# BlackCloud37/rust-raytracer

Hardware: AMD Instinct MI355X
Metric: Msamples/sec (px*spp), scene_500 1200x1200 1000spp (higher is better)
Workload: dtype f64

## Files before the change

### rust-raytracer_amd/csrc/device/kernels.hip

```cpp
#include <hip/hip_runtime.h>

#include <cmath>
#include <cstdio>
#include <chrono>
#include <cstdlib>
#include <cstring>
#include <map>
#include <memory>
#include <mutex>
#include <vector>

#include "../common/flat.h"
#include "../common/grid_shape.h"
#include "../common/detlog.h"
#include "../common/detsin.h"
#include "../common/detuv.h"
#include "../common/rng.h"
#include "../common/schedule.h"
#include "../common/tighten.h"
#include "device.h"

namespace rtamd {

#ifndef PT_BLOCK
#define PT_BLOCK 1024
#endif

#define HIP_CHECK(expr)                                                                                  \
    do {                                                                                                 \
        hipError_t _e = (expr);                                                                          \
        if (_e != hipSuccess)                                                                            \
            throw RtError((_e == hipErrorNoDevice || _e == hipErrorInvalidDevice) ? RT_ERR_NO_DEVICE : RT_ERR_HIP, \
                          std::string(#expr) + ": " + hipGetErrorString(_e));                            \
    } while (0)

#ifdef RTAMD_PHASE_STATS
__shared__ unsigned long long s_ph[48];
__device__ unsigned long long g_phase[48];
__device__ __forceinline__ bool ph_first() { return (int)(__ffsll((long long)__ballot(1)) - 1) == (int)(threadIdx.x & 63); }
#define PH_CLK() __builtin_amdgcn_s_memtime()
#define PH_ADD(i, dt)                                                         \
    do {                                                                      \
        if (ph_first()) atomicAdd(&s_ph[(i)], (unsigned long long)(dt));      \
    } while (0)
#define PH_EV(i)                                                              \
    do {                                                                      \
        const unsigned long long _m = __ballot(1);                            \
        if (ph_first()) {                                                     \
            atomicAdd(&s_ph[16 + (i)], 1ull);                                 \
            atomicAdd(&s_ph[32 + (i)], (unsigned long long)__popcll(_m));     \
        }                                                                     \
    } while (0)
#define PH_BEGIN(v) const unsigned long long v = PH_CLK()
#define PH_END(i, v)              \
    do {                          \
        PH_ADD(i, PH_CLK() - v);  \
        PH_EV(i);                 \
    } while (0)
#else
#define PH_ADD(i, dt) \
    do {              \
    } while (0)
#define PH_EV(i) \
    do {         \
    } while (0)
#define PH_BEGIN(v) \
    do {            \
    } while (0)
#define PH_END(i, v) \
    do {             \
    } while (0)
#endif

struct D3 {
    double x, y, z;
};
#define DEV __device__ __forceinline__
DEV D3 mk(double x, double y, double z) { D3 r; r.x = x; r.y = y; r.z = z; return r; }
DEV D3 add(D3 a, D3 b) { return mk(a.x + b.x, a.y + b.y, a.z + b.z); }
DEV D3 sub(D3 a, D3 b) { return mk(a.x - b.x, a.y - b.y, a.z - b.z); }
DEV D3 muls(D3 a, double s) { return mk(a.x * s, a.y * s, a.z * s); }
DEV D3 divs(D3 a, double s) { return mk(a.x / s, a.y / s, a.z / s); }
DEV D3 neg(D3 a) { return mk(-a.x, -a.y, -a.z); }
DEV D3 elemul(D3 a, D3 b) { return mk(a.x * b.x, a.y * b.y, a.z * b.z); }
DEV double dot(D3 a, D3 b) { return a.x * b.x + a.y * b.y + a.z * b.z; }
DEV double sqlen(D3 a) { return a.x * a.x + a.y * a.y + a.z * a.z; }
DEV D3 cross(D3 a, D3 b) { return mk(a.y * b.z - a.z * b.y, a.z * b.x - a.x * b.z, a.x * b.y - a.y * b.x); }
DEV double comp(D3 a, int i) { return i == 0 ? a.x : (i == 1 ? a.y : a.z); }
DEV D3 unit(D3 a, int* err) {
    double l = sqrt(sqlen(a));
    if (l == 0.) atomicOr(err, 1);
    return divs(a, l);
}
DEV bool near_zero(D3 a) {
    const double S = 1e-8;
    return (fabs(a.x) < S) && (fabs(a.y) < S) && (fabs(a.z) < S);
}
DEV D3 reflect(D3 v, D3 n) { return sub(v, muls(n, 2. * dot(v, n))); }
DEV D3 refract(D3 uv, D3 n, double eta) {
    double cos_theta = fmin(dot(neg(uv), n), 1.0);
    D3 perp = muls(add(uv, muls(n, cos_theta)), eta);
    D3 par = muls(n, -sqrt(fabs(1.0 - sqlen(perp))));
    return add(perp, par);
}
DEV D3 random_in_unit_sphere(Rng& rng) {
    double u, v, r2;
    for (;;) {
        u = rng.gen_range_pm1();
        v = rng.gen_range_pm1();
        r2 = u * u + v * v;
        if (r2 <= 1.) break;
    }
    double q = sqrt(1. - r2);
    return mk(2. * u * q, 2. * v * q, 1. - 2. * r2);
}
DEV D3 random_in_unit_disk(Rng& rng) {
    for (;;) {
        double a = rng.gen_range_pm1();
        double b = rng.gen_range_pm1();
        if (a * a + b * b + 0. * 0. >= 1.) continue;
        return mk(a, b, 0.);
    }
}
DEV D3 xf_point(const double* t, D3 p) {
    return mk(t[0] * p.x + t[1] * p.y + t[2] * p.z + t[3] * 1., t[4] * p.x + t[5] * p.y + t[6] * p.z + t[7] * 1.,
              t[8] * p.x + t[9] * p.y + t[10] * p.z + t[11] * 1.);
}
DEV D3 xf_dir(const double* t, D3 p) {
    return mk(t[0] * p.x + t[1] * p.y + t[2] * p.z + t[3] * 0., t[4] * p.x + t[5] * p.y + t[6] * p.z + t[7] * 0.,
              t[8] * p.x + t[9] * p.y + t[10] * p.z + t[11] * 0.);
}

#define AS_G __attribute__((address_space(1)))
// ... 1342 lines not shown
    const AreaTriDev* k = T + lo;
    double u = x2, v = x3;
    if (u + v > 1.0) {
        u = 1.0 - u;
        v = 1.0 - v;
    }
    const D3 p = add(mk(k->a[0], k->a[1], k->a[2]), add(muls(mk(k->e0[0], k->e0[1], k->e0[2]), u), muls(mk(k->e1[0], k->e1[1], k->e1[2]), v)));
    return sub(p, o);
}
__device__ __attribute__((noinline)) double area_pdf(const char* tab, uint32_t li, D3 o, D3 d) {
    const AreaTab a = area_tab(tab);
    const AreaLightDev l = a.lights[li];
    const double total = (double)l.total, d2 = sqlen(d), dl = sqrt(d2);
    double sum = 0.0;
    for (uint32_t i = 0; i < l.count; i++) {
        const AreaTriDev* k = a.tris + l.first + i;
        double t, b1, b2;
        if (!tri_hit_v(mk(k->a[0], k->a[1], k->a[2]), mk(k->e0[0], k->e0[1], k->e0[2]), mk(k->e1[0], k->e1[1], k->e1[2]), o, d, 0.001, INFINITY, t, b1, b2)) continue;
        const double area2 = k->area2;
        const double dist2 = (t * t) * d2;
        const double cosine = fabs(dot(d, mk(k->n[0], k->n[1], k->n[2])) / (dl * area2));
        if (!(cosine > 0.)) continue;
        sum = sum + (((double)k->q / total) * dist2) / (cosine * (0.5 * area2));
    }
    return sum;
}
DEV bool mixture_step_area(const Acc& A, const char* area, const char* env, const Rec& rec, Rng& rng, D3 att, D3& beta, D3& dir, int* err) {
    const double PI = 3.14159265358979323846264338327950288;
    const uint32_t M = ((const AreaHdr*)area)->n_lights;
    const uint32_t n = A.n_lights + M + (env ? 1u : 0u);
    if (rng.gen_f64() < 0.5) {
        uint32_t li = (uint32_t)(rng.gen_f64() * (double)n);
        if (li >= n) li = n - 1u;
        if (li < A.n_lights) {
            dir = light_random(A, A.lights[li], rec.p, rng, err);
        } else if (li < A.n_lights + M) {
            const double x1 = rng.gen_f64(), x2 = rng.gen_f64(), x3 = rng.gen_f64();
            dir = area_sample(area, li - A.n_lights, rec.p, x1, x2, x3);
        } else {
            const double x1 = rng.gen_f64(), x2 = rng.gen_f64(), x3 = rng.gen_f64(), x4 = rng.gen_f64();
            dir = env_sample(env, x1, x2, x3, x4);
        }
    }
    double cosine = dot(rec.normal, unit(dir, err));
    double scattering_pdf = (cosine < 0.) ? 0. : cosine / PI;
    double lp = 0.;
    for (uint32_t i = 0; i < A.n_lights; i++) lp = lp + light_pdf_value(A, A.lights[i], rec.p, dir);
    for (uint32_t i = 0; i < M; i++) lp = lp + area_pdf(area, i, rec.p, dir);
    if (env) lp = lp + env_pdf(env, dir, err);
    double pdf_val = 0.5 * (lp / (double)n) + 0.5 * scattering_pdf;
    double wgt = scattering_pdf / pdf_val;
    if (!(wgt > 0.)) return false;
    beta = muls(elemul(beta, att), wgt);
    return true;
}

#ifndef REGEN_MIN
#define REGEN_MIN 8
#endif
#ifndef FOLD_RETRY
#define FOLD_RETRY 4
#endif
#ifndef COOP_EARLY_FOLD
#define COOP_EARLY_FOLD 1
#endif
#ifndef POOL_MODE
#define POOL_MODE 1
#endif
#ifndef FOLD_BATCH
#define FOLD_BATCH 1
#endif
#ifndef FOLD_PERIOD
#define FOLD_PERIOD 4
#endif
#ifndef UNIT_SPP_N
#define UNIT_SPP_N 8
#endif
static const int UNIT_SPP = UNIT_SPP_N;
#ifndef RING_UNITS
#define RING_UNITS 8
#endif
static const int UNIT_DOUBLES = UNIT_SPP * TILE_PIX * 3;
static_assert(RING_UNITS * 4 <= 64, "a wave clears its ring bookkeeping with one store per lane");
#ifndef SINGLE_UNITS_BELOW_WAVES
#define SINGLE_UNITS_BELOW_WAVES 1
#endif
#ifndef JOB_UNITS
#define JOB_UNITS 2
#endif
DEV uint64_t ld_agent(const uint64_t* p) { return __hip_atomic_load(p, __ATOMIC_RELAXED, __HIP_MEMORY_SCOPE_AGENT); }
DEV void st_agent(uint64_t* p, uint64_t v) { __hip_atomic_store(p, v, __ATOMIC_RELAXED, __HIP_MEMORY_SCOPE_AGENT); }
DEV uint64_t ld_agent_g(const AS_G uint64_t* p) { return __hip_atomic_load(p, __ATOMIC_RELAXED, __HIP_MEMORY_SCOPE_AGENT); }
DEV void st_agent_g(AS_G uint64_t* p, uint64_t v) { __hip_atomic_store(p, v, __ATOMIC_RELAXED, __HIP_MEMORY_SCOPE_AGENT); }

#ifdef RT_TAIL_STATS
__device__ unsigned long long g_tail_end[8192], g_tail_beg[8192], g_tail_entry[8192];
__device__ unsigned int g_tail_xcc[8192];
#endif
#ifdef RT_FOLD_STATS
__device__ unsigned long long g_fold_stats[8];
#endif
__device__ __attribute__((noinline)) int fold_units(const uint32_t* rmeta, const double* wring, double* accum, unsigned int* tickets, bool first_launch,
                                                    int r_head, int r_cnt, bool idle, int lane, int ring_units) {
#ifdef RT_FOLD_STATS
    const unsigned long long t_in = __builtin_amdgcn_s_memtime();
    unsigned long long n_mis = 0, n_sleep = 0;
#endif
    const AS_L uint32_t* rm = (const AS_L uint32_t*)rmeta;
    AS_G unsigned int* tk_g = (AS_G unsigned int*)tickets;
    int folded = 0;
    bool have = false;
    uint32_t cur_tile = 0;
    double ax = 0., ay = 0., az = 0.;
    asm volatile("s_waitcnt vmcnt(0)" ::: "memory");
    while (r_cnt > 0) {
        const AS_L uint32_t* m = rm + 4 * r_head;
        if (__hip_atomic_load(&m[3], __ATOMIC_RELAXED, __HIP_MEMORY_SCOPE_WORKGROUP) != 0u) break;
        const uint32_t tile = m[0], blk = m[1], ns = m[2] & 0xffu;
        const bool first = (m[2] & 0x100u) != 0u, last = (m[2] & 0x200u) != 0u;
        if (first) {
            const uint32_t tk = __hip_atomic_load(&tk_g[tile], __ATOMIC_RELAXED, __HIP_MEMORY_SCOPE_AGENT);
            if (tk != blk) {
#ifdef RT_FOLD_STATS
                if (!idle) n_mis++;
                else n_sleep++;
#endif
                if (!idle) break;
                __builtin_amdgcn_s_sleep(4);
                continue;
            }
        }
        AS_G uint64_t* acc = (AS_G uint64_t*)accum + ((size_t)tile * TILE_PIX + (size_t)lane) * 3;
        if (!have) {
            ax = 0.; ay = 0.; az = 0.;
            if (!(blk == 0u && first_launch)) {
                ax = __longlong_as_double(ld_agent_g(acc));
                ay = __longlong_as_double(ld_agent_g(acc + 1));
                az = __longlong_as_double(ld_agent_g(acc + 2));
            }
            have = true;
            cur_tile = tile;
        }
        const AS_G uint64_t* p = (const AS_G uint64_t*)wring + ((size_t)r_head * UNIT_SPP * TILE_PIX + (size_t)lane) * 3;
        uint32_t si = 0;
#if FOLD_BATCH > 1
        for (; si + FOLD_BATCH <= ns; si += FOLD_BATCH) {
            uint64_t v[3 * FOLD_BATCH];
#pragma unroll
            for (int k = 0; k < 3 * FOLD_BATCH; k++) v[k] = ld_agent_g(p + (size_t)(k / 3) * (TILE_PIX * 3) + (k % 3));
#pragma unroll
            for (int j = 0; j < FOLD_BATCH; j++) {
                ax = ax + __longlong_as_double(v[3 * j]);
                ay = ay + __longlong_as_double(v[3 * j + 1]);
                az = az + __longlong_as_double(v[3 * j + 2]);
            }
            p += FOLD_BATCH * TILE_PIX * 3;
        }
#endif
        for (; si < ns; si++) {
            const uint64_t v0 = ld_agent_g(p), v1 = ld_agent_g(p + 1), v2 = ld_agent_g(p + 2);
            ax = ax + __longlong_as_double(v0);
            ay = ay + __longlong_as_double(v1);
            az = az + __longlong_as_double(v2);
            p += TILE_PIX * 3;
        }
        r_head = (r_head + 1 == ring_units) ? 0 : r_head + 1;
// ... 259 lines not shown
}

#ifndef RT_TIGHTEN_BOXES
#define RT_TIGHTEN_BOXES 1
#endif
static constexpr int INTEG_BG = 4;
static constexpr int INTEG_ENV = 8;
static constexpr int INTEG_AREA = 16;
template <bool LDS, int GENERAL, int ACCEL, int INTEG, bool MEDIA = false, bool POOL = false>
__global__ void __launch_bounds__(PT_BLOCK) pt_kernel(FlatView sv, CamK cam, RenderK rk, double* __restrict__ ring, double* accum,
                                                      unsigned int* tickets, unsigned int* __restrict__ counter, int* __restrict__ err) {
    extern __shared__ __attribute__((aligned(16))) char smem[];
#ifdef RT_TAIL_STATS
    const unsigned long long tail_entry = __builtin_amdgcn_s_memrealtime();
#endif
    const uint32_t st_begin = (ACCEL == 2) ? sv.stage2_begin : 0u;
    const uint32_t st_end = (ACCEL == 2) ? sv.stage2_end : sv.stage_bytes;
    uint32_t staged = 0;
    Acc A;
    if (LDS && ACCEL == 2) {
        const uint32_t lo_bytes = sv.off_n2 - st_begin;
        {
            const uint4* src = (const uint4*)(sv.base + st_begin);
            uint4* dst = (uint4*)smem;
            for (uint32_t i = threadIdx.x; i < lo_bytes / 16; i += blockDim.x) dst[i] = src[i];
        }
        char* n2w = smem + lo_bytes;
        stage_nodew(sv, n2w, rk.box_shrink);
        staged = lo_bytes + nodew_bytes(sv.n_nodes2);
        __syncthreads();
        A = make_acc(smem - st_begin, sv.base, sv);
        A.n2 = nullptr;
        A.n2w_lds = (uint32_t)(uintptr_t)(AS_L char*)n2w;
        if (MEDIA) {
            A.meta = (const uint2*)(sv.base + sv.off_meta);
            A.boxes = (const double2*)(sv.base + sv.off_boxes);
        }
    } else if (LDS) {
        const uint4* src = (const uint4*)(sv.base + st_begin);
        uint4* dst = (uint4*)smem;
        for (uint32_t i = threadIdx.x; i < (st_end - st_begin) / 16; i += blockDim.x) dst[i] = src[i];
        staged = st_end - st_begin;
        __syncthreads();
        A = make_acc(smem - st_begin, sv.base, sv);
    } else {
        A = make_acc(sv.base, sv.base, sv);
        if (ACCEL == 2 && rk.n_top > 0) {
            const uint4* src = (const uint4*)(sv.base + sv.off_n2);
            uint4* dst = (uint4*)smem;
            for (uint32_t i = threadIdx.x; i < (uint32_t)rk.n_top * NODE2_F4; i += blockDim.x) dst[i] = src[i];
            __syncthreads();
            A.n2_top = (const AS_L f32x4*)smem;
            A.n2_top_count = (uint32_t)rk.n_top;
            staged = (uint32_t)rk.n_top * (uint32_t)sizeof(Node2);
        }
    }
    const char* area_env = nullptr;
    if ((INTEG & INTEG_AREA) && sv.off_env != 0u && ((const EnvTabHdr*)(sv.base + sv.total_bytes))->total != 0ull) area_env = sv.base + sv.total_bytes;
    uint32_t* stk = (uint32_t*)(smem + staged) + threadIdx.x;
    const int stk_stride = (int)blockDim.x;
    const int lane = threadIdx.x & 63;
    const uint64_t lanemask_lt = (1ull << lane) - 1ull;
    const int wave = threadIdx.x >> 6;
    uint32_t* book = (uint32_t*)(smem + staged + walk_stack_bytes((ACCEL == 2) ? sv.stack2 : 0u, PT_BLOCK));
    uint32_t* rmeta = book + (size_t)wave * RING_UNITS * 4;
    uint32_t* wst = book + (size_t)(PT_BLOCK / 64) * RING_UNITS * 4 + (size_t)wave * 8;
    int* cfg = (int*)(book + (size_t)(PT_BLOCK / 64) * (RING_UNITS * 4 + 8));
    if (lane < 8) wst[lane] = (lane == 6) ? 1u : 0u;
    if (POOL && lane < RING_UNITS * 4) rmeta[lane] = 0u;
    if (threadIdx.x == 0) {
        cfg[CFG_N_JOBS] = rk.n_units; cfg[CFG_TILES_OWNED] = rk.tiles_owned; cfg[CFG_JOB_UNITS] = rk.job_units;
        cfg[CFG_SUBS_PER_TILE] = rk.subs_per_tile; cfg[CFG_WORLD] = rk.world; cfg[CFG_RANK] = rk.rank; cfg[CFG_TILES_X] = rk.tiles_x;
        cfg[CFG_S_BEGIN] = rk.s_begin; cfg[CFG_S_END] = rk.s_end; cfg[CFG_SUB_SPP] = rk.sub_spp; cfg[CFG_WIDTH] = rk.width;
        cfg[CFG_HEIGHT] = rk.height;
        cfg[CFG_RING_UNITS] = RING_UNITS;
        cfg[CFG_JOB_LISTS] = 1;
#pragma unroll
        for (int i = 0; i < 25; i++) cfg[CFG_LVL + i] = rk.lvl[i / 5][i % 5];
        cfg[CFG_TILE_LIST] = (int)(uint32_t)(uintptr_t)rk.tile_list; cfg[CFG_TILE_LIST + 1] = (int)(uint32_t)((uint64_t)(uintptr_t)rk.tile_list >> 32);
    }
    if (GENERAL >= 2 && rk.time_slots) A.time_lds = (uint32_t)(uintptr_t)(AS_L char*)(cfg + CFG_WORDS);
    __syncthreads();
    double* wring = ring + ((size_t)blockIdx.x * (PT_BLOCK / 64) + (size_t)wave) * RING_UNITS * UNIT_DOUBLES;

    int tx = 0, ty = 0, s0 = 0, pool = 0, next = 0, cur_slot = 0;
    bool finished = false;

    bool alive = false;
    D3 o = mk(0, 0, 0), d = mk(0, 0, 1), beta = mk(1, 1, 1), L = mk(0, 0, 0);
    int depth = 0;
    int pix_id = 0;
    uint32_t out_slot = 0;
    Rng rng;
    rng.s = 0;
#ifdef RT_TAIL_STATS
    const unsigned long long tail_t0 = __builtin_amdgcn_s_memrealtime();
#endif
    int fold_wait = 0;
#ifdef RTAMD_PHASE_STATS
    if (threadIdx.x < 48) s_ph[threadIdx.x] = 0ull;
    __syncthreads();
#endif
    {
        for (;;) {
            PH_BEGIN(ph_it0);
            uint64_t dead = __ballot(!alive);
            if ((int)__popcll(dead) < REGEN_MIN && dead != ~0ull) dead = 0ull;
            const bool need_unit = dead != 0ull && next >= pool && !finished;
            bool head_ready = false;
            if (FOLD_PERIOD > 0 && !need_unit && --fold_wait < 0) {
                fold_wait = FOLD_PERIOD - 1;
                head_ready = __builtin_amdgcn_readfirstlane(wst[1]) != 0u &&
                             __builtin_amdgcn_readfirstlane(__hip_atomic_load(&rmeta[4 * __builtin_amdgcn_readfirstlane(wst[0]) + 3], __ATOMIC_RELAXED,
                                                                              __HIP_MEMORY_SCOPE_WORKGROUP)) == 0u;
            }
            if (need_unit || head_ready) {
                const UnitInfo u = uniform_unit(POOL ? next_unit_pool(wst, rmeta, cfg, wring, accum, tickets, counter, need_unit && dead == ~0ull, lane, need_unit)
                                                     : next_unit(wst, rmeta, cfg, wring, accum, tickets, counter, need_unit && dead == ~0ull, lane, need_unit));
                if (need_unit) {
                    if (u.pool > 0) {
                        pool = u.pool;
                        next = 0;
                        s0 = u.s0;
                        tx = u.tx;
                        ty = u.ty;
                        cur_slot = u.cur_slot;
                    }
                    finished = u.finished != 0;
                } else if (u.cur_slot == 0) {
                    fold_wait = FOLD_RETRY;
                }
            }
            if (dead != 0ull && next < pool) {
                int k = next + __popcll(dead & lanemask_lt);
                next = min(next + (int)__popcll(dead), pool);
                if (!alive && k < pool) {
                    int pix = k & (TILE_PIX - 1), s = s0 + (k >> 6);
                    int x = tx * TILE_W + (pix & (TILE_W - 1)), y = ty * TILE_H + (pix >> 3);
                    if (x < rk.width && y < rk.height) {
                        rng.seed_stream(rk.seed, (uint64_t)y * (uint64_t)rk.width + (uint64_t)x, (uint64_t)s);
                        double u = ((double)x + rng.gen_f64()) / (double)(rk.width - 1);
                        double v = ((double)y + rng.gen_f64()) / (double)(rk.height - 1);
                        double st = 1.0 - v;
                        D3 rd = muls(random_in_unit_disk(rng), cam.lens_radius);
                        if (GENERAL >= 2 && rk.time1 > rk.time0) {
                            const double tm = rng.gen_range(rk.time0, rk.time1);
                            if (A.time_lds) *(AS_L double*)(uintptr_t)(A.time_lds + 8u * threadIdx.x) = tm;
                        } else if (GENERAL >= 2 && A.time_lds) {
                            *(AS_L double*)(uintptr_t)(A.time_lds + 8u * threadIdx.x) = rk.time0;
                        }
                        D3 offset = add(muls(cam.u, rd.x), muls(cam.v, rd.y));
                        o = add(cam.origin, offset);
                        d = sub(sub(add(add(cam.llc, muls(cam.horizontal, u)), muls(cam.vertical, st)), cam.origin), offset);
                        beta = mk(1., 1., 1.);
                        L = mk(0., 0., 0.);
                        depth = rk.max_depth;
                        pix_id = y * rk.width + x;
                        out_slot = ((uint32_t)cur_slot * (uint32_t)UNIT_SPP + (uint32_t)(k >> 6)) * (uint32_t)TILE_PIX + (uint32_t)pix;
                        alive = true;
                    }
                }
            }
            PH_END(0, ph_it0);
            if (__ballot(alive) == 0ull && next >= pool && finished) break;
            if (alive) {
                PH_EV(13);
                PH_BEGIN(ph_t0);
                Hit h = (ACCEL == 2) ? (MEDIA ? traverse2_media<GENERAL, !LDS, LDS>(A, sv.n_media, stk, stk_stride, o, d, rk.t_min, rng)
                                              : traverse2<GENERAL, false, !LDS, LDS>(A, stk, stk_stride, o, d, rk.t_min, INFINITY))
                                     : traverse<GENERAL, MEDIA>(A, o, d, rk.t_min, INFINITY, &rng);
                PH_END(1, ph_t0);
                PH_BEGIN(ph_p0);
                bool done = true;
                if (h.node >= 0 && depth > 0) {
                    depth -= 1;
                    PH_BEGIN(ph_m0);
                    const Rec rec = materialize<GENERAL>(A, h, o, d, err);
                    PH_END(2, ph_m0);
                    constexpr bool SEG_IN_PLACE = !(GENERAL == 1 && !LDS && ACCEL == 2 && INTEG == INTEG_BG && MEDIA) &&
                                                  !(GENERAL == 3 && LDS && ACCEL == 1 && INTEG == (INTEG_BG | 1));
                    if (SEG_IN_PLACE) o = rec.p;
                    D3 emitted, att, ndir = d;
                    D3& nd = SEG_IN_PLACE ? d : ndir;
                    bool diffuse, scattered;
                    PH_BEGIN(ph_s0);
                    if constexpr (GENERAL == 0) {
                        const auto add_emitted = [&](const D3& le) {
                            L = add(L, elemul(beta, le));
                            asm volatile("" : "+v"(L.x), "+v"(L.y), "+v"(L.z));
                        };
                        scattered = shade<GENERAL>(A, rec, d, rng, emitted, att, nd, diffuse, err, add_emitted);
                    } else {
                        scattered = shade<GENERAL>(A, rec, d, rng, emitted, att, nd, diffuse, err);
                        L = add(L, elemul(beta, emitted));
                    }
                    PH_END(3, ph_s0);
                    if (scattered) {
                        if ((INTEG & 3) == 2 && diffuse) {
                            const double* e = rk.sppm_est + 6 * (size_t)pix_id;
                            L = add(L, elemul(beta, mk(e[0], e[1], e[2])));
                            L = add(L, elemul(beta, mk(e[3], e[4], e[5])));
                        } else if ((INTEG & 3) == 1 && diffuse) {
                            PH_EV(14);
                            if (INTEG & INTEG_AREA) done = !mixture_step_area(A, sv.base + sv.off_area, area_env, rec, rng, att, beta, nd, err);
                            else if (INTEG & INTEG_ENV) done = !mixture_step_env(A, sv.base + sv.total_bytes, rec, rng, att, beta, nd, err);
                            else done = !mixture_step(A, rec, rng, att, beta, nd, err);
                        } else {
                            beta = elemul(beta, att);
                            done = false;
                        }
                        if (!SEG_IN_PLACE && !done) {
                            o = rec.p;
                            d = ndir;
                        }
                    }
                } else if ((INTEG & INTEG_BG) && h.node < 0 && (!(INTEG & INTEG_AREA) || sv.off_bg != 0u)) {
                    L = add(L, elemul(beta, background_radiance<GENERAL>((const BgDev*)(sv.base + sv.off_bg), A.texs, A.texels, d, err)));
                }
                if (done) {
                    double* dst = wring + 3 * (size_t)out_slot;
                    dst[0] = L.x;
                    dst[1] = L.y;
                    dst[2] = L.z;
                    atomicSub(rmeta + 4 * (out_slot >> 9) + 3, 1u);
                    alive = false;
                }
                PH_END(8, ph_p0);
            }
        }
    }
#ifdef RTAMD_PHASE_STATS
    __syncthreads();
    if (threadIdx.x < 48) atomicAdd(&g_phase[threadIdx.x], s_ph[threadIdx.x]);
#endif
#ifdef RT_TAIL_STATS
    if (lane == 0) {
        g_tail_end[blockIdx.x * (PT_BLOCK / 64) + wave] = __builtin_amdgcn_s_memrealtime();
        g_tail_beg[blockIdx.x * (PT_BLOCK / 64) + wave] = tail_t0;
        g_tail_entry[blockIdx.x * (PT_BLOCK / 64) + wave] = tail_entry;
        g_tail_xcc[blockIdx.x * (PT_BLOCK / 64) + wave] = 0u;
    }
#endif
}

#ifndef COOP_POOL
#define COOP_POOL 1024
#endif
#define COOP_RING (2 * COOP_POOL)
static_assert(COOP_RING >= 2 * COOP_POOL && COOP_POOL <= 32768 && (COOP_RING & (COOP_RING - 1)) == 0,
              "kernel 5's rings: 16-bit entries (id + 1), power-of-two capacity of at least twice the pool (see ring_pop)");
#ifndef COOP_SPIN_MAX
#define COOP_SPIN_MAX (1u << 16)
#endif
#ifndef COOP_BATCH
#define COOP_BATCH 32
#endif
#ifndef COOP_REFILL_TH
#define COOP_REFILL_TH 56
#endif
#ifndef COOP_ENTRY_NODES
#define COOP_ENTRY_NODES 64
#endif
#ifndef COOP_ADOPT_MIN
#define COOP_ADOPT_MIN 8
#endif
#ifndef COOP_SUSPEND_TH
#define COOP_SUSPEND_TH 24
#endif
static const int COOP_MAX_INST = 64;
static const int COOP_STACK_MAX = 40;
static const int COOP_REC = 20 + COOP_STACK_MAX / 2 + 2;
typedef unsigned long long U2 __attribute__((ext_vector_type(2)));
DEV U2 ld_unit(const uint64_t* rec, int unit) { return ((const U2*)rec)[unit]; }
DEV void st_unit(uint64_t* rec, int unit, uint64_t a, uint64_t b) {
    U2 v;
    v.x = a;
    v.y = b;
    ((U2*)rec)[unit] = v;
}
DEV uint64_t dbits(double x) { return (uint64_t)__double_as_longlong(x); }
DEV double bitsd(uint64_t x) { return __longlong_as_double((long long)x); }

#ifdef RTAMD_COOP_STATS
__device__ unsigned long long g_coop_stats[16];
struct CoopStats {
    unsigned long long ev[8] = {0, 0, 0, 0, 0, 0, 0, 0}, ln[8] = {0, 0, 0, 0, 0, 0, 0, 0};
    unsigned long long tm[8] = {0, 0, 0, 0, 0, 0, 0, 0}, t_last = 0;
};
__device__ unsigned long long g_coop_time[8];
#define COOP_RING_T0 const unsigned long long t_ring0 = __builtin_amdgcn_s_memtime()
#define COOP_RING_T1 cs.tm[7] += __builtin_amdgcn_s_memtime() - t_ring0
#define COOP_TIME(i)                                                      \
    do {                                                                  \
        const unsigned long long t_now = __builtin_amdgcn_s_memtime();    \
        cs.tm[i] += t_now - cs.t_last;                                    \
        cs.t_last = t_now;                                                \
    } while (0)
#define COOP_STATS_ARG , CoopStats& cs
#define COOP_STATS_PASS , cs
#define COOP_STAT(i, lanes_mask)                                        \
    do {                                                                \
        cs.ev[i] += 1ull;                                               \
        cs.ln[i] += (unsigned long long)__popcll(lanes_mask);           \
    } while (0)
#else
#define COOP_STATS_ARG
#define COOP_STATS_PASS
#define COOP_STAT(i, lanes_mask) \
    do {                         \
    } while (0)
#define COOP_TIME(i) \
    do {             \
    } while (0)
#define COOP_RING_T0
#define COOP_RING_T1
#endif
// ... 1558 lines not shown
    if (kernel == 0)
        kernel = accel2_usable ? ((coop_usable && view.max_inst_nodes2 >= 64u) ? 5 : (wf_usable && !coop_usable && view.max_inst_nodes2 >= 64u) ? 6 : 2) : 1;
    if (kernel == 5 && !coop_usable)
        throw RtError(RT_ERR_UNSUPPORTED, "kernel 5 (cooperative instance service) needs a usable accel, 1..64 instances of which at least one holds only triangles with f32 vertices (an OBJ mesh), of BVH depth <= 40");
    if (kernel == 6 && !wf_usable)
        throw RtError(RT_ERR_UNSUPPORTED, "kernel 6 (wavefront instance service) needs a usable accel and 1..64 instances of which at least one holds only triangles with f32 vertices (an OBJ mesh)");
    if ((kernel == 2 || kernel == 5) && !accel2_usable)
        throw RtError(RT_ERR_UNSUPPORTED, "kernel 2 requested but no usable accel for this scene/camera (unbounded item, depth overflow, stacks "
                                          "larger than LDS, negative t_min, or camera farther than 64x the scene extent); use kernel 0/1");
    c.kernel = kernel;
    const size_t ring_meta = ((size_t)(PT_BLOCK / 64) * (RING_UNITS * 4 + 8) + CFG_WORDS) * sizeof(uint32_t);
    c.stack_bytes = ((kernel == 2) ? stack2_bytes : (kernel == 5) ? stack5_bytes : 0) + ring_meta + ((kernel == 5) ? coop_lds : 0);
    if (plan.tile_list && !plan.ext_accum) throw RtError(RT_ERR_INTERNAL, "a tile list needs the caller's (compact) accumulator");
    if (plan.ext_accum && (kernel == 6 || plan.integrator == 2))
        throw RtError(RT_ERR_UNSUPPORTED, "resumable rendering (rt_render_accumulate_device) runs with kernels 1 / 2 / 5 and integrators 0 / 1");
    const int integ = plan.integrator;
    if (integ == 1 && view.n_lights == 0 && (kernel == 6 || (!c.env && !area))) throw RtError(RT_ERR_ARG, "integrator 1 (light importance sampling) needs rt_scene_set_lights");
    if (integ == 2 && !plan.sppm_est) throw RtError(RT_ERR_ARG, "integrator 2 (SPPM) is reached through rt_render_sppm");
    if (kernel == 6) return c;
    const size_t nodew = ((size_t)(view.n_nodes2 + NODEW_CHUNK - 1) / NODEW_CHUNK) * 3 * NODEW_FAR;
    c.hot_bytes = (kernel == 2 || kernel == 5) ? hot2 - (size_t)view.n_nodes2 * sizeof(Node2) + nodew : hot1;
    c.lds = c.hot_bytes > 0 && c.hot_bytes + c.stack_bytes <= lds_max && !tun.no_lds && kernel != 5;
    if (integ != 0 && book2)
        throw RtError(RT_ERR_UNSUPPORTED, "the book-2 extensions (moving spheres, noise textures, an open shutter) render with integrator 0 (kernels 1 and 2)");
    if (media && integ == 1)
        throw RtError(RT_ERR_UNSUPPORTED, "scenes with a ConstantMedium render with integrator 0 only (the medium's random draw is part of the "
                                          "reference-order walk; light sampling and SPPM have no volume events)");
    if (nest && kernel != 1 && kernel != 2) throw RtError(RT_ERR_INTERNAL, "nested Transforms reached kernel " + std::to_string(kernel));
    return c;
}

struct LaunchLayout {
    pt_fn fn = nullptr;
    pt_coop_fn fn_coop = nullptr;
    int n_top = 0, n_topq = 0;
    size_t smem = 0;
    int grid = 0;
    bool pool = false;
    float node_shrink = 0.f;
    int64_t n_pix = 0;
    size_t ring_bytes = 0, accum_bytes = 0, ticket_bytes = 0, coop_bytes = 0;
    size_t workspace_bytes = 0;
};
static LaunchLayout launch_layout(const FlatView& view, const RenderPlan& plan, const Tuning& tun, const DevInfo& di, const KernelChoice& c) {
    LaunchLayout L;
    const int kernel = c.kernel, integ = plan.integrator;
    const size_t lds_max = c.lds_max, stack_bytes = c.stack_bytes;
    if (kernel == 2 && !c.lds && lds_max > stack_bytes) {
        size_t room = (lds_max - stack_bytes) / sizeof(Node2);
        if (tun.n_top >= 0) room = std::min<size_t>(room, (size_t)tun.n_top);
        L.n_top = (int)std::min<size_t>(room, view.n_nodes2);
    }
    if (kernel == 5 && lds_max > stack_bytes) {
        size_t room = lds_max - stack_bytes;
        L.n_top = (int)std::min<size_t>(std::min<size_t>(room / sizeof(Node2), 128), view.world_top2);
        if (tun.n_top >= 0) L.n_top = std::min(L.n_top, tun.n_top);
        room -= (size_t)L.n_top * sizeof(Node2);
        L.n_topq = (int)std::min<size_t>(room / sizeof(NodeQ), view.n_nodes2);
        if (tun.n_top >= 0) L.n_topq = std::min(L.n_topq, tun.n_top);
    }
    const size_t smem = L.smem = (c.lds ? c.hot_bytes : (size_t)L.n_top * sizeof(Node2) + (size_t)L.n_topq * sizeof(NodeQ)) + stack_bytes +
                                 (c.variant.moving ? (size_t)PT_BLOCK * sizeof(double) : 0);
    const bool early = kernel == 5 && COOP_EARLY_FOLD && plan.tiles_owned < (int64_t)2 * di.cus * (PT_BLOCK / 64);
    if (kernel == 5)
        L.fn_coop = coop_variant(CoopKey{integ, view.n_inline2 != 0u || view.n_inst2 > 32u, early, view.n_inst2 > 32u, tie_scene(view)});
    else
        L.fn = pt_variant(pt_key(c, integ, false));
    const void* fptr = (kernel == 5) ? (const void*)L.fn_coop : (const void*)L.fn;
    if (smem > 48 * 1024) HIP_CHECK(hipFuncSetAttribute(fptr, hipFuncAttributeMaxDynamicSharedMemorySize, (int)smem));
    int blocks_per_cu = 0;
    HIP_CHECK(hipOccupancyMaxActiveBlocksPerMultiprocessor(&blocks_per_cu, fptr, PT_BLOCK, smem));
    if (blocks_per_cu < 1) blocks_per_cu = 1;
    const int grid = L.grid = di.cus * blocks_per_cu;
    const SceneVariant& v = c.variant;
    L.pool = POOL_MODE && SINGLE_UNITS_BELOW_WAVES && plan.tiles_owned < (int64_t)grid * (PT_BLOCK / 64) &&
             ((kernel == 2 && !v.media && !v.book2 && !v.nest && !c.bg && !c.area) || (kernel == 5 && early));
    if (L.pool && kernel == 2) {
        L.fn = pt_variant(pt_key(c, integ, true));
        if (smem > 48 * 1024) HIP_CHECK(hipFuncSetAttribute((const void*)L.fn, hipFuncAttributeMaxDynamicSharedMemorySize, (int)smem));
    }
    L.node_shrink = (RT_TIGHTEN_BOXES && kernel == 2 && c.lds) ? box_shrink(view.origin_limit2, render_origin_bound(view.origin_limit2, c.cam_abs), view.n_inst2 == 0u) : 0.f;
    L.n_pix = plan.tiles_owned * TILE_PIX;
    L.ring_bytes = (size_t)grid * (PT_BLOCK / 64) * RING_UNITS * UNIT_DOUBLES * sizeof(double);
    L.accum_bytes = std::max<size_t>(16, (size_t)L.n_pix * 3 * sizeof(double));
    L.ticket_bytes = std::max<size_t>(16, (size_t)plan.tiles_owned * sizeof(unsigned int));
    L.coop_bytes = (kernel == 5) ? (size_t)grid * COOP_POOL * COOP_REC * sizeof(uint64_t) : 0;
    L.workspace_bytes = L.ring_bytes + (size_t)L.n_pix * 3 * sizeof(double) + (size_t)plan.tiles_owned * sizeof(unsigned int) + L.coop_bytes;
    return L;
}

static void fill_stats(rt_stats* st, const rt_scene& s, const RenderPlan& plan, int kernel, bool lds, int grid, double kernel_ms, int launches, size_t workspace_bytes) {
    if (!st) return;
    st->kernel_ms = kernel_ms;
    st->reduce_ms = 0.;
    st->launches = launches;
    st->kernel_used = kernel;
    st->scene_in_lds = lds ? 1 : 0;
    st->block_threads = PT_BLOCK;
    st->grid_blocks = grid;
    st->spp_chunk = plan.spp_chunk;
    st->scene_bytes = s.flat.blob.size();
    st->reserved[1] = (uint64_t)workspace_bytes;
}

static void print_tool_stats(int kernel, bool lds, int grid, const rt_stats* st, int launches = 0, int grid_w = 0, uint32_t seg = 0, uint32_t n_topq_w = 0) {
#ifdef RTAMD_WF_STATS
    if (kernel == 6) {
        unsigned long long hs[16], z[16] = {0};
        HIP_CHECK(hipMemcpyFromSymbol(hs, HIP_SYMBOL(g_wf_stats), sizeof(hs)));
        const char* names[12] = {"parks", "adoptions", "generated", "wave iterations", "wave exits: ring full / no unit", "wave exits: gate closed", "wave exits: finished",
                                 "wave cycles in launches", "alive lanes summed", "entry walks", "walk passes", "walk pass lanes"};
        fprintf(stderr, "[wf stats] cycles %d  grid %d x %d  walk grid %d  seg %u  n_topq_w %u\n", launches, grid, PT_BLOCK, grid_w, seg, n_topq_w);
        for (int i = 0; i < 12; i++) fprintf(stderr, "[wf stats] %-34s %14llu\n", names[i], hs[i]);
        HIP_CHECK(hipMemcpyToSymbol(HIP_SYMBOL(g_wf_stats), z, sizeof(z)));
    }
#endif
    if (kernel == 6) return;
#ifdef RTAMD_COOP_STATS
    if (kernel == 5) {
        unsigned long long hs[16], z[16] = {0};
        HIP_CHECK(hipMemcpyFromSymbol(hs, HIP_SYMBOL(g_coop_stats), sizeof(hs)));
        const char* names[8] = {"serve rounds (lanes at start)", "serve passes (busy lanes)", "walk phases (lanes)", "shade phases (lanes)", "suspensions (walks)", "idle sleeps", "adoptions (paths)", "... that hit inside the instance"};
        for (int i = 0; i < 8; i++)
            fprintf(stderr, "[coop stats] %-32s %12llu  lanes %14llu  (%.1f per event)\n", names[i], hs[2 * i], hs[2 * i + 1],
                    hs[2 * i] ? (double)hs[2 * i + 1] / (double)hs[2 * i] : 0.);
        HIP_CHECK(hipMemcpyToSymbol(HIP_SYMBOL(g_coop_stats), z, sizeof(z)));
        unsigned long long tm[8], tot = 0;
        HIP_CHECK(hipMemcpyFromSymbol(tm, HIP_SYMBOL(g_coop_time), sizeof(tm)));
        for (int i = 0; i < 7; i++) tot += tm[i];
        const char* tn[8] = {"fold + regenerate", "world-space walk", "park", "adopt", "shade", "serve (batch)", "tail: serve rest / idle", "(of park + adopt: the two ring pops)"};
        for (int i = 0; i < 8; i++) fprintf(stderr, "[coop time] %-26s %5.1f %%\n", tn[i], tot ? 100. * (double)tm[i] / (double)tot : 0.);
        HIP_CHECK(hipMemcpyToSymbol(HIP_SYMBOL(g_coop_time), z, sizeof(tm)));
    }
#endif
#ifdef RTAMD_PHASE_STATS
    if (kernel != 5) {
        unsigned long long hp[48], z[48] = {0};
        HIP_CHECK(hipMemcpyFromSymbol(hp, HIP_SYMBOL(g_phase), sizeof(hp)));
        HIP_CHECK(hipMemcpyToSymbol(HIP_SYMBOL(g_phase), z, sizeof(z)));
        const double tot = (double)(hp[0] + hp[1] + hp[8]);
        const char* nm[16] = {"regeneration", "traverse (all)", "materialize", "shade (all)", "  Lambertian / light branch", "  Isotropic branch", "  Metal branch",
                              "  Dielectric branch", "after traverse (all)", "  leaf sections of traverse", "inner-node steps", "leaf items", "cube tests",
                              "segments", "mixture steps", "  node steps inside an instance"};
        fprintf(stderr, "[phase] kernel %d lds %d  wave clocks per segment-iteration %.0f (iterations %llu)\n", kernel, lds ? 1 : 0, hp[16] ? tot / (double)hp[16] : 0.,
                hp[16]);
        for (int i = 0; i < 16; i++)
            fprintf(stderr, "[phase] %-30s time %6.3f  wave-exec/iter %8.3f  lanes/exec %5.1f  (util %.3f)\n", nm[i], i < 10 ? (double)hp[i] / tot : 0.,
                    hp[16] ? (double)hp[16 + i] / (double)hp[16] : 0., hp[16 + i] ? (double)hp[32 + i] / (double)hp[16 + i] : 0.,
                    hp[16 + i] ? (double)hp[32 + i] / (64. * (double)hp[16 + i]) : 0.);
        double save = 0.;
        for (int i = 4; i <= 7; i++)
            if (hp[16 + i]) save += (double)hp[i] * (1. - (double)hp[32 + i] / (64. * (double)hp[16 + i]));
        fprintf(stderr, "[phase] material branches: %.4f of wave time; re-binned to full waves they would return at most %.4f\n",
                (double)(hp[4] + hp[5] + hp[6] + hp[7]) / tot, save / tot);
    }
#endif
#ifdef RT_TAIL_STATS
    if (kernel != 5 && st) {
        const int wpb = PT_BLOCK / 64, nw = grid * wpb;
        std::vector<unsigned long long> te(8192), tb(8192);
        HIP_CHECK(hipMemcpyFromSymbol(te.data(), HIP_SYMBOL(g_tail_end), sizeof(unsigned long long) * 8192));
        HIP_CHECK(hipMemcpyFromSymbol(tb.data(), HIP_SYMBOL(g_tail_beg), sizeof(unsigned long long) * 8192));
        std::vector<unsigned long long> tn(8192);
        std::vector<unsigned int> xc(8192);
        HIP_CHECK(hipMemcpyFromSymbol(xc.data(), HIP_SYMBOL(g_tail_xcc), sizeof(unsigned int) * 8192));
        HIP_CHECK(hipMemcpyFromSymbol(tn.data(), HIP_SYMBOL(g_tail_entry), sizeof(unsigned long long) * 8192));
        unsigned long long x0[8];
        for (int x = 0; x < 8; x++) x0[x] = ~0ull;
        for (int i = 0; i < nw; i++) x0[xc[i]] = std::min(x0[xc[i]], tn[i]);
        {
            std::vector<double> n(nw), sg(nw);
            for (int i = 0; i < nw; i++) { n[i] = (double)(tn[i] - x0[xc[i]]); sg[i] = (double)(tb[i] - tn[i]); }
            std::sort(n.begin(), n.end());
            std::sort(sg.begin(), sg.end());
            fprintf(stderr, "[tail stats] (ticks) kernel entry after the XCD's first wave: 50%% %.0f  99%% %.0f  last %.0f; entry -> main loop (staging): 50%% %.0f  last %.0f\n", n[nw / 2],
                    n[nw * 99 / 100], n[nw - 1], sg[nw / 2], sg[nw - 1]);
        }
        std::vector<double> b(nw), e(nw);
        for (int i = 0; i < nw; i++) { b[i] = (double)(tb[i] - x0[xc[i]]); e[i] = (double)(te[i] - x0[xc[i]]); }
        std::sort(b.begin(), b.end());
        std::sort(e.begin(), e.end());
        const double k = st->kernel_ms / e[nw - 1];
        double idle = 0;
        for (int i = 0; i < nw; i++) idle += e[nw - 1] - e[i];
        fprintf(stderr, "[tail stats] kernel %.2f ms; wave starts: 50%% %.3f  99%% %.3f  last %.3f ms; wave ends: first %.2f  10%% %.2f  50%% %.2f  90%% %.2f  99%% %.2f  last %.2f ms; "
                        "mean idle wave-time at the end %.2f ms\n",
                st->kernel_ms, k * b[nw / 2], k * b[nw * 99 / 100], k * b[nw - 1], k * e[0], k * e[nw / 10], k * e[nw / 2], k * e[nw * 9 / 10], k * e[nw * 99 / 100],
                k * e[nw - 1], k * idle / nw);
    }
#endif
#ifdef RT_FOLD_STATS
    {
        unsigned long long hs[8], z[8] = {0};
        HIP_CHECK(hipMemcpyFromSymbol(hs, HIP_SYMBOL(g_fold_stats), sizeof(hs)));
        fprintf(stderr, "[fold stats] calls %llu  cycles %llu (%.0f per call)  units folded %llu  ticket mismatches %llu  sleeps %llu\n", hs[0], hs[1],
                hs[0] ? (double)hs[1] / (double)hs[0] : 0., hs[2], hs[3], hs[4]);
        HIP_CHECK(hipMemcpyToSymbol(HIP_SYMBOL(g_fold_stats), z, sizeof(z)));
    }
#endif
}

static void render_tiles_wf(const rt_scene& s, const FlatView& view, const CameraDev& cam, const RenderPlan& plan, const Tuning& tun, double* d_tiles,
                            hipStream_t stream, rt_stats* st, int dev, const DevInfo& di, const KernelChoice& c);

void render_tiles(const rt_scene& s, const CameraDev& cam, const RenderPlan& plan, double* d_tiles, void* stream_, rt_stats* st) {
    if (!s.committed) throw RtError(RT_ERR_NOT_COMMITTED, "scene not committed");
    const Tuning tun = tuning();
    hipStream_t stream = (hipStream_t)stream_;
    int dev = 0;
    HIP_CHECK(hipGetDevice(&dev));
    const DevInfo& di = dev_info(dev);

    FlatView view = s.flat.view;
    double upload_ms = 0.;
    uint64_t env_total = 0;
    view.base = device_blob(s, dev, &upload_ms, &env_total);
    if (st) st->upload_ms = upload_ms;
    const KernelChoice c = choose_kernel(s, view, cam, plan, tun, di, env_total);
    const int kernel = c.kernel;
    if (kernel == 6) {
        render_tiles_wf(s, view, cam, plan, tun, d_tiles, stream, st, dev, di, c);
        return;
    }
    const LaunchLayout lay = launch_layout(view, plan, tun, di, c);
    const int grid = lay.grid;
    WorkspaceLease lease(dev, lay.ring_bytes, lay.accum_bytes, lay.ticket_bytes, lay.coop_bytes);
    struct Ptr {
        void* p;
    };
    char* small = (char*)lease.w->small;
    Ptr ringp{lease.w->ring}, accum{plan.ext_accum ? (void*)plan.ext_accum : lease.w->accum}, tickets{lease.w->tickets}, counter{small}, err{small + 16};
    const int s_first = plan.ext_accum ? plan.s_first : 0, s_last = (plan.ext_accum && plan.s_last >= 0) ? plan.s_last : plan.spp;
    HIP_CHECK(hipMemsetAsync(small, 0, WS_SMALL, stream));
    Events events;
    std::vector<std::pair<hipEvent_t, hipEvent_t>> pt_ev;
// ... 697 lines not shown
```

Measured before the change: 3072.

## Batch camera-ray generation per sample row across full wave into scratch buffer

In the camera-regeneration path, when a wave starts a new 64-pixel sample row it now generates every camera ray of that row with all lanes in parallel. Each lane writes origin, direction and RNG state to a per-wave global scratch batch, and the dead lanes that later pick up those paths read them back. The aim is to avoid regenerating rays at low lane utilisation, where only the few dead lanes do the seeding, sampling and lens math. In exchange it adds global stores and loads, explicit vmcnt waits and a larger ring allocation, and it can compute rays that are not consumed right away. Phase-stats instrumentation gains a counter for the regeneration block.

```diff
diff --git a/rust-raytracer_amd/csrc/device/kernels.hip b/rust-raytracer_amd/csrc/device/kernels.hip
--- a/rust-raytracer_amd/csrc/device/kernels.hip
+++ b/rust-raytracer_amd/csrc/device/kernels.hip
@@ -35,8 +35,9 @@
     } while (0)
 
 #ifdef RTAMD_PHASE_STATS
-__shared__ unsigned long long s_ph[48];
-__device__ unsigned long long g_phase[48];
+#define PH_N 17
+__shared__ unsigned long long s_ph[3 * PH_N];
+__device__ unsigned long long g_phase[3 * PH_N];
 __device__ __forceinline__ bool ph_first() { return (int)(__ffsll((long long)__ballot(1)) - 1) == (int)(threadIdx.x & 63); }
 #define PH_CLK() __builtin_amdgcn_s_memtime()
 #define PH_ADD(i, dt)                                                         \
@@ -47,8 +48,8 @@
     do {                                                                      \
         const unsigned long long _m = __ballot(1);                            \
         if (ph_first()) {                                                     \
-            atomicAdd(&s_ph[16 + (i)], 1ull);                                 \
-            atomicAdd(&s_ph[32 + (i)], (unsigned long long)__popcll(_m));     \
+            atomicAdd(&s_ph[PH_N + (i)], 1ull);                                \
+            atomicAdd(&s_ph[2 * PH_N + (i)], (unsigned long long)__popcll(_m));    \
         }                                                                     \
     } while (0)
 #define PH_BEGIN(v) const unsigned long long v = PH_CLK()
@@ -1557,6 +1558,7 @@
 #endif
 static const int UNIT_DOUBLES = UNIT_SPP * TILE_PIX * 3;
 static_assert(RING_UNITS * 4 <= 64, "a wave clears its ring bookkeeping with one store per lane");
+static const int BATCH_DOUBLES = 4 * 2 * TILE_PIX;
 #ifndef SINGLE_UNITS_BELOW_WAVES
 #define SINGLE_UNITS_BELOW_WAVES 1
 #endif
@@ -1982,6 +1984,9 @@
     if (GENERAL >= 2 && rk.time_slots) A.time_lds = (uint32_t)(uintptr_t)(AS_L char*)(cfg + CFG_WORDS);
     __syncthreads();
     double* wring = ring + ((size_t)blockIdx.x * (PT_BLOCK / 64) + (size_t)wave) * RING_UNITS * UNIT_DOUBLES;
+    constexpr bool CAM_BATCH = LDS && GENERAL == 0 && ACCEL == 2 && !MEDIA;
+    double2* wbatch = (double2*)(ring + (size_t)gridDim.x * (PT_BLOCK / 64) * RING_UNITS * UNIT_DOUBLES +
+                                 ((size_t)blockIdx.x * (PT_BLOCK / 64) + (size_t)wave) * BATCH_DOUBLES);
 
     int tx = 0, ty = 0, s0 = 0, pool = 0, next = 0, cur_slot = 0;
     bool finished = false;
@@ -1998,7 +2003,7 @@
 #endif
     int fold_wait = 0;
 #ifdef RTAMD_PHASE_STATS
-    if (threadIdx.x < 48) s_ph[threadIdx.x] = 0ull;
+    if (threadIdx.x < 3 * PH_N) s_ph[threadIdx.x] = 0ull;
     __syncthreads();
 #endif
     {
@@ -2032,34 +2037,84 @@
                 }
             }
             if (dead != 0ull && next < pool) {
-                int k = next + __popcll(dead & lanemask_lt);
-                next = min(next + (int)__popcll(dead), pool);
-                if (!alive && k < pool) {
-                    int pix = k & (TILE_PIX - 1), s = s0 + (k >> 6);
-                    int x = tx * TILE_W + (pix & (TILE_W - 1)), y = ty * TILE_H + (pix >> 3);
-                    if (x < rk.width && y < rk.height) {
-                        rng.seed_stream(rk.seed, (uint64_t)y * (uint64_t)rk.width + (uint64_t)x, (uint64_t)s);
-                        double u = ((double)x + rng.gen_f64()) / (double)(rk.width - 1);
-                        double v = ((double)y + rng.gen_f64()) / (double)(rk.height - 1);
-                        double st = 1.0 - v;
-                        D3 rd = muls(random_in_unit_disk(rng), cam.lens_radius);
-                        if (GENERAL >= 2 && rk.time1 > rk.time0) {
-                            const double tm = rng.gen_range(rk.time0, rk.time1);
-                            if (A.time_lds) *(AS_L double*)(uintptr_t)(A.time_lds + 8u * threadIdx.x) = tm;
-                        } else if (GENERAL >= 2 && A.time_lds) {
-                            *(AS_L double*)(uintptr_t)(A.time_lds + 8u * threadIdx.x) = rk.time0;
+                const int k = next + __popcll(dead & lanemask_lt);
+                const int next_end = min(next + (int)__popcll(dead), pool);
+                if constexpr (CAM_BATCH) {
+                    int b = next >> 6;
+                    bool due = (next & 63) == 0;
+#pragma nounroll
+                    for (;;) {
+                        if (due) {
+                            const int gx = tx * TILE_W + (lane & (TILE_W - 1)), gy = ty * TILE_H + (lane >> 3);
+                            asm volatile("s_waitcnt vmcnt(0)" ::: "memory");
+                            if (gx < rk.width && gy < rk.height) {
+                                Rng g;
+                                g.seed_stream(rk.seed, (uint64_t)gy * (uint64_t)rk.width + (uint64_t)gx, (uint64_t)(s0 + b));
+                                const double u = ((double)gx + g.gen_f64()) / (double)(rk.width - 1);
+                                const double v = ((double)gy + g.gen_f64()) / (double)(rk.height - 1);
+                                const double st = 1.0 - v;
+                                const D3 rd = muls(random_in_unit_disk(g), cam.lens_radius);
+                                const D3 offset = add(muls(cam.u, rd.x), muls(cam.v, rd.y));
+                                const D3 go = add(cam.origin, offset);
+                                const D3 gd = sub(sub(add(add(cam.llc, muls(cam.horizontal, u)), muls(cam.vertical, st)), cam.origin), offset);
+                                wbatch[lane] = make_double2(go.x, go.y);
+                                wbatch[TILE_PIX + lane] = make_double2(go.z, gd.x);
+                                wbatch[2 * TILE_PIX + lane] = make_double2(gd.y, gd.z);
+                                wbatch[3 * TILE_PIX + lane] = make_double2(__longlong_as_double((long long)g.s), 0.);
+                            }
+                            asm volatile("s_waitcnt vmcnt(0)" ::: "memory");
                         }
-                        D3 offset = add(muls(cam.u, rd.x), muls(cam.v, rd.y));
-                        o = add(cam.origin, offset);
-                        d = sub(sub(add(add(cam.llc, muls(cam.horizontal, u)), muls(cam.vertical, st)), cam.origin), offset);
-                        beta = mk(1., 1., 1.);
-                        L = mk(0., 0., 0.);
-                        depth = rk.max_depth;
-                        pix_id = y * rk.width + x;
-                        out_slot = ((uint32_t)cur_slot * (uint32_t)UNIT_SPP + (uint32_t)(k >> 6)) * (uint32_t)TILE_PIX + (uint32_t)pix;
-                        alive = true;
+                        if (!alive && k < pool && (k >> 6) == b) {
+                            PH_EV(16);
+                            const int pix = k & (TILE_PIX - 1);
+                            const int x = tx * TILE_W + (pix & (TILE_W - 1)), y = ty * TILE_H + (pix >> 3);
+                            if (x < rk.width && y < rk.height) {
+                                const double2 e0 = wbatch[pix], e1 = wbatch[TILE_PIX + pix], e2 = wbatch[2 * TILE_PIX + pix], e3 = wbatch[3 * TILE_PIX + pix];
+                                o = mk(e0.x, e0.y, e1.x);
+                                d = mk(e1.y, e2.x, e2.y);
+                                rng.s = (uint64_t)__double_as_longlong(e3.x);
+                                beta = mk(1., 1., 1.);
+                                L = mk(0., 0., 0.);
+                                depth = rk.max_depth;
+                                pix_id = y * rk.width + x;
+                                out_slot = ((uint32_t)cur_slot * (uint32_t)UNIT_SPP + (uint32_t)b) * (uint32_t)TILE_PIX + (uint32_t)pix;
+                                alive = true;
+                            }
+                        }
+                        b += 1;
+                        due = true;
+                        if ((b << 6) >= next_end) break;
+                    }
+                } else {
+                    if (!alive && k < pool) {
+                        PH_EV(16);
+                        int pix = k & (TILE_PIX - 1), s = s0 + (k >> 6);
+                        int x = tx * TILE_W + (pix & (TILE_W - 1)), y = ty * TILE_H + (pix >> 3);
+                        if (x < rk.width && y < rk.height) {
+                            rng.seed_stream(rk.seed, (uint64_t)y * (uint64_t)rk.width + (uint64_t)x, (uint64_t)s);
+                            double u = ((double)x + rng.gen_f64()) / (double)(rk.width - 1);
+                            double v = ((double)y + rng.gen_f64()) / (double)(rk.height - 1);
+                            double st = 1.0 - v;
+                            D3 rd = muls(random_in_unit_disk(rng), cam.lens_radius);
+                            if (GENERAL >= 2 && rk.time1 > rk.time0) {
+                                const double tm = rng.gen_range(rk.time0, rk.time1);
+                                if (A.time_lds) *(AS_L double*)(uintptr_t)(A.time_lds + 8u * threadIdx.x) = tm;
+                            } else if (GENERAL >= 2 && A.time_lds) {
+                                *(AS_L double*)(uintptr_t)(A.time_lds + 8u * threadIdx.x) = rk.time0;
+                            }
+                            D3 offset = add(muls(cam.u, rd.x), muls(cam.v, rd.y));
+                            o = add(cam.origin, offset);
+                            d = sub(sub(add(add(cam.llc, muls(cam.horizontal, u)), muls(cam.vertical, st)), cam.origin), offset);
+                            beta = mk(1., 1., 1.);
+                            L = mk(0., 0., 0.);
+                            depth = rk.max_depth;
+                            pix_id = y * rk.width + x;
+                            out_slot = ((uint32_t)cur_slot * (uint32_t)UNIT_SPP + (uint32_t)(k >> 6)) * (uint32_t)TILE_PIX + (uint32_t)pix;
+                            alive = true;
+                        }
                     }
                 }
+                next = next_end;
             }
             PH_END(0, ph_it0);
             if (__ballot(alive) == 0ull && next >= pool && finished) break;
@@ -2131,7 +2186,7 @@
     }
 #ifdef RTAMD_PHASE_STATS
     __syncthreads();
-    if (threadIdx.x < 48) atomicAdd(&g_phase[threadIdx.x], s_ph[threadIdx.x]);
+    if (threadIdx.x < 3 * PH_N) atomicAdd(&g_phase[threadIdx.x], s_ph[threadIdx.x]);
 #endif
 #ifdef RT_TAIL_STATS
     if (lane == 0) {
@@ -3856,6 +3911,7 @@
     L.node_shrink = (RT_TIGHTEN_BOXES && kernel == 2 && c.lds) ? box_shrink(view.origin_limit2, render_origin_bound(view.origin_limit2, c.cam_abs), view.n_inst2 == 0u) : 0.f;
     L.n_pix = plan.tiles_owned * TILE_PIX;
     L.ring_bytes = (size_t)grid * (PT_BLOCK / 64) * RING_UNITS * UNIT_DOUBLES * sizeof(double);
+    if (kernel == 2 && c.lds && pt_key(c, integ, false).general == 0 && !v.media) L.ring_bytes += (size_t)grid * (PT_BLOCK / 64) * BATCH_DOUBLES * sizeof(double);
     L.accum_bytes = std::max<size_t>(16, (size_t)L.n_pix * 3 * sizeof(double));
     L.ticket_bytes = std::max<size_t>(16, (size_t)plan.tiles_owned * sizeof(unsigned int));
     L.coop_bytes = (kernel == 5) ? (size_t)grid * COOP_POOL * COOP_REC * sizeof(uint64_t) : 0;
@@ -3909,22 +3965,22 @@
 #endif
 #ifdef RTAMD_PHASE_STATS
     if (kernel != 5) {
-        unsigned long long hp[48], z[48] = {0};
+        unsigned long long hp[3 * PH_N], z[3 * PH_N] = {0};
         HIP_CHECK(hipMemcpyFromSymbol(hp, HIP_SYMBOL(g_phase), sizeof(hp)));
         HIP_CHECK(hipMemcpyToSymbol(HIP_SYMBOL(g_phase), z, sizeof(z)));
+        const unsigned long long *hw = hp + PH_N, *hl = hp + 2 * PH_N;
         const double tot = (double)(hp[0] + hp[1] + hp[8]);
-        const char* nm[16] = {"regeneration", "traverse (all)", "materialize", "shade (all)", "  Lambertian / light branch", "  Isotropic branch", "  Metal branch",
-                              "  Dielectric branch", "after traverse (all)", "  leaf sections of traverse", "inner-node steps", "leaf items", "cube tests",
-                              "segments", "mixture steps", "  node steps inside an instance"};
-        fprintf(stderr, "[phase] kernel %d lds %d  wave clocks per segment-iteration %.0f (iterations %llu)\n", kernel, lds ? 1 : 0, hp[16] ? tot / (double)hp[16] : 0.,
-                hp[16]);
-        for (int i = 0; i < 16; i++)
+        const char* nm[PH_N] = {"regeneration", "traverse (all)", "materialize", "shade (all)", "  Lambertian / light branch", "  Isotropic branch", "  Metal branch",
+                                "  Dielectric branch", "after traverse (all)", "  leaf sections of traverse", "inner-node steps", "leaf items", "cube tests",
+                                "segments", "mixture steps", "  node steps inside an instance", "regeneration block (paths taken)"};
+        fprintf(stderr, "[phase] kernel %d lds %d  wave clocks per segment-iteration %.0f (iterations %llu)\n", kernel, lds ? 1 : 0, hw[0] ? tot / (double)hw[0] : 0.,
+                hw[0]);
+        for (int i = 0; i < PH_N; i++)
             fprintf(stderr, "[phase] %-30s time %6.3f  wave-exec/iter %8.3f  lanes/exec %5.1f  (util %.3f)\n", nm[i], i < 10 ? (double)hp[i] / tot : 0.,
-                    hp[16] ? (double)hp[16 + i] / (double)hp[16] : 0., hp[16 + i] ? (double)hp[32 + i] / (double)hp[16 + i] : 0.,
-                    hp[16 + i] ? (double)hp[32 + i] / (64. * (double)hp[16 + i]) : 0.);
+                    hw[0] ? (double)hw[i] / (double)hw[0] : 0., hw[i] ? (double)hl[i] / (double)hw[i] : 0., hw[i] ? (double)hl[i] / (64. * (double)hw[i]) : 0.);
         double save = 0.;
         for (int i = 4; i <= 7; i++)
-            if (hp[16 + i]) save += (double)hp[i] * (1. - (double)hp[32 + i] / (64. * (double)hp[16 + i]));
+            if (hw[i]) save += (double)hp[i] * (1. - (double)hl[i] / (64. * (double)hw[i]));
         fprintf(stderr, "[phase] material branches: %.4f of wave time; re-binned to full waves they would return at most %.4f\n",
                 (double)(hp[4] + hp[5] + hp[6] + hp[7]) / tot, save / tot);
     }
```

Result: faster. 3130 (median of 6 runs) (+1.9%).
